# vitskvara/VBMatrixFactorization.jl

Hardware: AMD Instinct MI355X
Metric: VB iterations/sec (higher is better)
Workload: dtype bf16

## Files before the change

### vbmatrixfactorization.jl_amd/csrc/gram_kernels.hpp

```cpp
#pragma once
#include "common.hpp"
#include "ctrl_kernels.hpp"
#include "post_kernels.hpp"

namespace vbmf {

#ifndef GRAM_CHUNK
#define GRAM_CHUNK 256
#endif
constexpr int GRAM_PLANES = 5;
constexpr long long GRAM_G_NT_BYTES = 240LL << 20;

__device__ __forceinline__ unsigned pack_bf2(unsigned short lo, unsigned short hi) { return (unsigned)lo | ((unsigned)hi << 16); }

__global__ __launch_bounds__(256) void gram_build_kernel(const uint4* __restrict__ Y1, int XT, int KS, float* __restrict__ Gt,
                                                         int GT) {
    const int P = blockIdx.y, Q = blockIdx.x;
    if (P > Q) return;
    const int lane = threadIdx.x & 63, w = threadIdx.x >> 6;
    const int p0 = 4 * P + 2 * (w >> 1), q0 = 4 * Q + 2 * (w & 1);
    const long long KT = 2LL * GT;
    double g64[2][2][16];
#pragma unroll
    for (int a = 0; a < 2; ++a)
#pragma unroll
        for (int b = 0; b < 2; ++b)
#pragma unroll
            for (int r = 0; r < 16; ++r) g64[a][b][r] = 0.0;
    const uint4 z = make_uint4(0u, 0u, 0u, 0u);
    const uint4* pa[2];
    const uint4* pb[2];
    bool oka[2], okb[2];
#pragma unroll
    for (int i = 0; i < 2; ++i) {
        oka[i] = p0 + i < XT; okb[i] = q0 + i < XT;
        pa[i] = Y1 + ((long long)(oka[i] ? p0 + i : 0) * KS) * 64 + lane;
        pb[i] = Y1 + ((long long)(okb[i] ? q0 + i : 0) * KS) * 64 + lane;
    }
    constexpr int U = 4;
    for (int k0 = 0; k0 < KS; k0 += GRAM_CHUNK) {
        const int k1 = min(k0 + GRAM_CHUNK, KS);
        f32x16 acc[2][2];
#pragma unroll
        for (int a = 0; a < 2; ++a)
#pragma unroll
            for (int b = 0; b < 2; ++b)
#pragma unroll
                for (int r = 0; r < 16; ++r) acc[a][b][r] = 0.f;
        for (int ks = k0; ks < k1; ks += U) {
            uint4 fa[U][2], fb[U][2];
#pragma unroll
            for (int u = 0; u < U; ++u) {
                const bool in = ks + u < k1;
#pragma unroll
                for (int i = 0; i < 2; ++i) {
                    fa[u][i] = (in && oka[i]) ? pa[i][(long long)(ks + u) * 64] : z;
                    fb[u][i] = (in && okb[i]) ? pb[i][(long long)(ks + u) * 64] : z;
                }
            }
#pragma unroll
            for (int u = 0; u < U; ++u)
#pragma unroll
                for (int a = 0; a < 2; ++a)
#pragma unroll
                    for (int b = 0; b < 2; ++b)
                        acc[a][b] = __builtin_amdgcn_mfma_f32_32x32x16_bf16(__builtin_bit_cast(bf16x8, fa[u][a]),
                                                                            __builtin_bit_cast(bf16x8, fb[u][b]), acc[a][b], 0, 0, 0);
        }
#pragma unroll
        for (int a = 0; a < 2; ++a)
#pragma unroll
            for (int b = 0; b < 2; ++b)
#pragma unroll
                for (int r = 0; r < 16; ++r) g64[a][b][r] += (double)acc[a][b][r];
    }
    const int half = lane >> 5, c = lane & 31;
#pragma unroll
    for (int a = 0; a < 2; ++a)
#pragma unroll
        for (int b = 0; b < 2; ++b) {
            const int p = p0 + a, q = q0 + b;
            if (p > q) continue;
#pragma unroll
            for (int r = 0; r < 16; ++r) {
                const int i = rho(r, half);
                const float v = (float)g64[a][b][r];
                Gt[(((long long)p * KT + 2 * q + (c >> 4)) * 64 + 32 * ((c >> 3) & 1) + i) * 8 + (c & 7)] = v;
                if (p != q) Gt[(((long long)q * KT + 2 * p + (i >> 4)) * 64 + 32 * ((i >> 3) & 1) + c) * 8 + (i & 7)] = v;
            }
        }
}

constexpr int GW_KS = 2, GW_ROWS = 16 * GW_KS;
template <int HP>
__global__ __launch_bounds__(HP * 4) void gram_w_kernel(const float* __restrict__ A32, const float* __restrict__ S,
                                                        const float* __restrict__ Wold, float* __restrict__ Wnew,
                                                        uint4* __restrict__ Wt, long long M, int KT, const int* __restrict__ stop) {
    if (*stop) return;
    constexpr int NS = HP / 16, NH = HP / 32, NT = HP * 4;
    __shared__ float sW[GW_ROWS][HP + 1];
    const int lane = threadIdx.x & 63, cb = threadIdx.x >> 6;
    const int q = lane >> 4, c = lane & 15;
    const long long row0 = (long long)blockIdx.x * GW_ROWS;
    double sb[NS][4];
#pragma unroll
    for (int s = 0; s < NS; ++s)
#pragma unroll
        for (int t = 0; t < 4; ++t) sb[s][t] = (double)S[(long long)(16 * s + 4 * q + t) * HP + 16 * cb + c];
#pragma unroll
    for (int mb = 0; mb < GW_KS; ++mb) {
        const long long m = row0 + 16 * mb + c;
        float4 a[NS];
#pragma unroll
        for (int s = 0; s < NS; ++s)
            a[s] = m < M ? *reinterpret_cast<const float4*>(A32 + m * HP + 16 * s + 4 * q) : make_float4(0.f, 0.f, 0.f, 0.f);
        f64x4 acc = {0.0, 0.0, 0.0, 0.0};
#pragma unroll
        for (int s = 0; s < NS; ++s) {
            acc = __builtin_amdgcn_mfma_f64_16x16x4f64((double)a[s].x, sb[s][0], acc, 0, 0, 0);
            acc = __builtin_amdgcn_mfma_f64_16x16x4f64((double)a[s].y, sb[s][1], acc, 0, 0, 0);
            acc = __builtin_amdgcn_mfma_f64_16x16x4f64((double)a[s].z, sb[s][2], acc, 0, 0, 0);
            acc = __builtin_amdgcn_mfma_f64_16x16x4f64((double)a[s].w, sb[s][3], acc, 0, 0, 0);
        }
#pragma unroll
        for (int r = 0; r < 4; ++r) sW[16 * mb + q + 4 * r][16 * cb + c] = (float)acc[r];
    }
    __syncthreads();
    const long long plane = (long long)KT * NH * 64;
    for (int it = threadIdx.x; it < GW_KS * NH * 64; it += NT) {
        const int jj = it / (NH * 64), ht = (it / 64) % NH, ln = it & 63;
        const int half = ln >> 5, h = 32 * ht + (ln & 31);
        const long long j = (long long)blockIdx.x * GW_KS + jj;
        if (j >= KT) continue;
        unsigned short wp[3][8], dp[2][8];
#pragma unroll
        for (int e = 0; e < 8; ++e) {
            const long long m = 16 * j + 8 * half + e;
            const float wv = sW[16 * jj + 8 * half + e][h];
            const float dv = (float)((double)wv - (double)Wold[m * HP + h]);
            Wnew[m * HP + h] = wv;
            wp[0][e] = f2bf(wv);
            float res = wv - bf2f(wp[0][e]);
            wp[1][e] = f2bf(res);
            res -= bf2f(wp[1][e]);
            wp[2][e] = f2bf(res);
            dp[0][e] = f2bf(dv);
            dp[1][e] = f2bf(dv - bf2f(dp[0][e]));
        }
        const long long o = (j * NH + ht) * 64 + ln;
#pragma unroll
        for (int p = 0; p < 3; ++p)
            Wt[p * plane + o] = make_uint4(pack_bf2(wp[p][0], wp[p][1]), pack_bf2(wp[p][2], wp[p][3]), pack_bf2(wp[p][4], wp[p][5]),
                                           pack_bf2(wp[p][6], wp[p][7]));
#pragma unroll
        for (int p = 0; p < 2; ++p)
            Wt[(3 + p) * plane + o] = make_uint4(pack_bf2(dp[p][0], dp[p][1]), pack_bf2(dp[p][2], dp[p][3]), pack_bf2(dp[p][4], dp[p][5]),
                                                 pack_bf2(dp[p][6], dp[p][7]));
    }
}

template <int HP, int NCG>
__global__ __launch_bounds__(HP * 4 / NCG) void gram_w_cols_kernel(const float* __restrict__ A32, const float* __restrict__ S,
                                                                   const float* __restrict__ Wold, float* __restrict__ Wnew,
                                                                   uint4* __restrict__ Wt, long long M, int KT,
                                                                   const int* __restrict__ stop) {
    if (*stop) return;
    constexpr int NS = HP / 16, NH = HP / 32, HC = HP / NCG, NHC = NH / NCG, NT = HP * 4 / NCG;
    static_assert(HC % 32 == 0 && NT <= 512, "gram_w_cols geometry");
    __shared__ float sW[GW_ROWS][HC + 1];
    const int lane = threadIdx.x & 63, cb = threadIdx.x >> 6;
    const int q = lane >> 4, c = lane & 15;
    const int col0 = blockIdx.y * HC;
    const long long row0 = (long long)blockIdx.x * GW_ROWS;
    double sb[NS][4];
#pragma unroll
    for (int s = 0; s < NS; ++s)
#pragma unroll
        for (int t = 0; t < 4; ++t) sb[s][t] = (double)S[(long long)(16 * s + 4 * q + t) * HP + col0 + 16 * cb + c];
#pragma unroll
    for (int mb = 0; mb < GW_KS; ++mb) {
        const long long m = row0 + 16 * mb + c;
        f64x4 acc = {0.0, 0.0, 0.0, 0.0};
#pragma unroll
        for (int s = 0; s < NS; ++s) {
            const float4 a = m < M ? *reinterpret_cast<const float4*>(A32 + m * HP + 16 * s + 4 * q) : make_float4(0.f, 0.f, 0.f, 0.f);
            acc = __builtin_amdgcn_mfma_f64_16x16x4f64((double)a.x, sb[s][0], acc, 0, 0, 0);
            acc = __builtin_amdgcn_mfma_f64_16x16x4f64((double)a.y, sb[s][1], acc, 0, 0, 0);
            acc = __builtin_amdgcn_mfma_f64_16x16x4f64((double)a.z, sb[s][2], acc, 0, 0, 0);
            acc = __builtin_amdgcn_mfma_f64_16x16x4f64((double)a.w, sb[s][3], acc, 0, 0, 0);
        }
#pragma unroll
        for (int r = 0; r < 4; ++r) sW[16 * mb + q + 4 * r][16 * cb + c] = (float)acc[r];
    }
    __syncthreads();
    const long long plane = (long long)KT * NH * 64;
    for (int it = threadIdx.x; it < GW_KS * NHC * 64; it += NT) {
        const int jj = it / (NHC * 64), htl = (it / 64) % NHC, ln = it & 63;
        const int half = ln >> 5, hl = 32 * htl + (ln & 31), h = col0 + hl, ht = blockIdx.y * NHC + htl;
        const long long j = (long long)blockIdx.x * GW_KS + jj;
        if (j >= KT) continue;
        unsigned short wp[3][8], dp[2][8];
#pragma unroll
        for (int e = 0; e < 8; ++e) {
            const long long m = 16 * j + 8 * half + e;
            const float wv = sW[16 * jj + 8 * half + e][hl];
            const float dv = (float)((double)wv - (double)Wold[m * HP + h]);
            Wnew[m * HP + h] = wv;
            wp[0][e] = f2bf(wv);
            float res = wv - bf2f(wp[0][e]);
            wp[1][e] = f2bf(res);
            res -= bf2f(wp[1][e]);
            wp[2][e] = f2bf(res);
            dp[0][e] = f2bf(dv);
            dp[1][e] = f2bf(dv - bf2f(dp[0][e]));
        }
        const long long o = (j * NH + ht) * 64 + ln;
#pragma unroll
        for (int p = 0; p < 3; ++p)
            Wt[p * plane + o] = make_uint4(pack_bf2(wp[p][0], wp[p][1]), pack_bf2(wp[p][2], wp[p][3]), pack_bf2(wp[p][4], wp[p][5]),
                                           pack_bf2(wp[p][6], wp[p][7]));
#pragma unroll
        for (int p = 0; p < 2; ++p)
            Wt[(3 + p) * plane + o] = make_uint4(pack_bf2(dp[p][0], dp[p][1]), pack_bf2(dp[p][2], dp[p][3]), pack_bf2(dp[p][4], dp[p][5]),
                                                 pack_bf2(dp[p][6], dp[p][7]));
    }
}

__device__ __forceinline__ float sub_f32(float a, float b) {
    float r;
    asm("v_sub_f32 %0, %1, %2" : "=v"(r) : "v"(a), "v"(b));
    return r;
}
__device__ __forceinline__ unsigned cvt_pk_bf16(float lo, float hi) {
    typedef __attribute__((ext_vector_type(2))) float f32x2v;
    typedef __attribute__((ext_vector_type(2))) __bf16 bf16x2v;
    const f32x2v v = {lo, hi};
    return __builtin_bit_cast(unsigned, __builtin_convertvector(v, bf16x2v));
}
__device__ __forceinline__ void split3_frag(const f32x4& x0, const f32x4& x1, u32x4v& g0, u32x4v& g1, u32x4v& g2) {
    const float v[8] = {x0.x, x0.y, x0.z, x0.w, x1.x, x1.y, x1.z, x1.w};
#pragma unroll
    for (int e = 0; e < 4; ++e) {
        float a = v[2 * e], b = v[2 * e + 1];
        const unsigned p0 = cvt_pk_bf16(a, b);
        a = sub_f32(a, bitsf(p0 << 16));
        b = sub_f32(b, bitsf(p0 & 0xffff0000u));
        const unsigned p1 = cvt_pk_bf16(a, b);
        a = sub_f32(a, bitsf(p1 << 16));
        b = sub_f32(b, bitsf(p1 & 0xffff0000u));
        g0[e] = p0;
        g1[e] = p1;
        g2[e] = cvt_pk_bf16(a, b);
    }
}

__device__ __forceinline__ f32x16 mfma_bf(const u32x4v& a, const u32x4v& b, const f32x16& c) {
    return __builtin_amdgcn_mfma_f32_32x32x16_bf16(__builtin_bit_cast(bf16x8, a), __builtin_bit_cast(bf16x8, b), c, 0, 0, 0);
}

#ifndef VBMF_GRAMPROD_PROBE
#define VBMF_GRAMPROD_PROBE 0
#endif
template <int NH>
struct GramProd {
    static constexpr int NW = 8;
    static constexpr int THREADS = 64 * NW;
    static constexpr int TPG = 16 / NH;
    static constexpr int NXW = TPG >= NW ? TPG / NW : 1;
    static constexpr int HS = TPG >= NW ? 1 : NW / TPG;
    static constexpr int NHW = NH / HS;
    static constexpr int CH = NH == 2 ? 4 : 2;
    static constexpr int D = 4;
    static constexpr int U = CH;
    static constexpr int NP = GRAM_PLANES * CH * NH;
    static constexpr int PPW = (NP + NW - 1) / NW;
    static constexpr int GL = 2 * NXW;
    static constexpr int GQ = VBMF_GRAMPROD_PROBE == 2 ? 0 : GL;
    static constexpr int PLANE_BYTES = 2 * NP * 1024;
    static constexpr int RING_BYTES = NW * D * GL * 1024;
    static constexpr int LDS_BYTES = PLANE_BYTES + RING_BYTES;
    static_assert(NXW * (NW / HS) == TPG && NHW * HS == NH, "gram_prod geometry");
    static_assert(LDS_BYTES <= 160 * 1024, "gram_prod LDS");
    static constexpr int g_wait(int u) {
        int n = (D - 1) * GQ;
        for (int d = 1; d < D; ++d) n += ((u + CH * D - d) % CH == 0) ? PPW : 0;
        return n;
    }
};
template <int NH, int NHT = NH>
__global__ __launch_bounds__(GramProd<NH>::THREADS) void gram_prod_kernel(const float4* __restrict__ Gt, const uint4* __restrict__ Wt,
                                                                          float* __restrict__ Out, int GT, int XT1, int sps, int nrg,
                                                                          long long n, long long slab_floats,
                                                                          const int* __restrict__ stop) {
    using C = GramProd<NH>;
    constexpr int NW = C::NW, NXW = C::NXW, NHW = C::NHW, D = C::D, CH = C::CH, U = C::U, NP = C::NP, PPW = C::PPW, GL = C::GL;
    extern __shared__ __attribute__((aligned(1024))) unsigned char gram_lds[];
    if (*stop) return;
    const int lane = threadIdx.x & 63;
    const int w = __builtin_amdgcn_readfirstlane(threadIdx.x >> 6);
    const int rg = blockIdx.x % nrg, s = blockIdx.x / nrg;
    const int KT = 2 * GT;
    const int j0 = s * sps, j1 = min(j0 + sps, KT), nk = j1 - j0;
    const int pt0 = rg * C::TPG + (w % (C::TPG / NXW)) * NXW;
    const int h0 = (w / (C::TPG / NXW)) * NHW;
    const int hg0 = NHT == NH ? 0 : (int)blockIdx.y * NH;
    const long long plane = (long long)KT * NHT * 64;
    f32x16 accP[NXW][NHW], accQ[NXW][NHW];
#pragma unroll
    for (int i = 0; i < NXW; ++i)
#pragma unroll
        for (int h = 0; h < NHW; ++h)
#pragma unroll
            for (int r = 0; r < 16; ++r) { accP[i][h][r] = 0.f; accQ[i][h][r] = 0.f; }
    __amdgpu_buffer_rsrc_t gr[NXW];
#pragma unroll
    for (int i = 0; i < NXW; ++i)
        gr[i] = __builtin_amdgcn_make_buffer_rsrc((void*)(Gt + (long long)(pt0 + i) * KT * 128), 0,
                                                  VBMF_GRAMPROD_PROBE == 1 ? 0u : (unsigned)KT * 2048u, 0x00020000);
    const __amdgpu_buffer_rsrc_t wr = __builtin_amdgcn_make_buffer_rsrc((void*)Wt, 0, (unsigned)(GRAM_PLANES * plane * 16), 0x00020000);
    const int voff = lane * 16;
    unsigned char* const ring = gram_lds + C::PLANE_BYTES + w * (D * GL * 1024);
    const bool g_nt = !(NH == 4 && NHT == 4) && (long long)GT * GT * 4096 > GRAM_G_NT_BYTES;
    auto load_g = [&](int slot, int t) __attribute__((always_inline)) {
        const int so = VBMF_GRAMPROD_PROBE == 3 ? 0 : min(j0 + t, j1 - 1) * 2048;
        if (g_nt) {
#pragma unroll
            for (int i = 0; i < NXW; ++i) {
                lds_dma_piece_nt(gr[i], ring + (slot * GL + 2 * i) * 1024, voff, so);
                lds_dma_piece_nt(gr[i], ring + (slot * GL + 2 * i + 1) * 1024, voff, so + 1024);
            }
        } else {
#pragma unroll
            for (int i = 0; i < NXW; ++i) {
                lds_dma_piece(gr[i], ring + (slot * GL + 2 * i) * 1024, voff, so);
                lds_dma_piece(gr[i], ring + (slot * GL + 2 * i + 1) * 1024, voff, so + 1024);
            }
        }
    };
    auto load_planes = [&](int cc, int t) __attribute__((always_inline)) {
#pragma unroll
        for (int v = 0; v < PPW; ++v) {
            const int x = min(w + NW * v, NP - 1);
            const int q = x / (CH * NH), r = x % (CH * NH);
            const int j = min(j0 + t + r / NH, j1 - 1);
            lds_dma_piece(wr, gram_lds + (cc * NP + x) * 1024, voff, (int)(q * plane + ((long long)j * NHT + hg0 + r % NH) * 64) * 16);
        }
    };
#pragma unroll
    for (int d = 0; d < D; ++d) {
        if ((d + CH * D - D) % CH == 0) load_planes(0, 0);
        load_g(d, d);
    }
    asm volatile("s_waitcnt vmcnt(%0)" ::"n"(CH * GL) : "memory");
    __builtin_amdgcn_s_barrier();
    asm volatile("" ::: "memory");
    u32x4v wf[GRAM_PLANES][NHW], g[NXW][3];
    auto mma = [&]() __attribute__((always_inline)) {
#pragma unroll
        for (int i = 0; i < NXW; ++i) {
#pragma unroll
            for (int h = 0; h < NHW; ++h) {
                f32x16 a = accP[i][h];
                a = mfma_bf(wf[2][h], g[i][0], a);
                a = mfma_bf(wf[1][h], g[i][1], a);
                a = mfma_bf(wf[0][h], g[i][2], a);
                a = mfma_bf(wf[1][h], g[i][0], a);
                a = mfma_bf(wf[0][h], g[i][1], a);
                accP[i][h] = mfma_bf(wf[0][h], g[i][0], a);
                f32x16 d = accQ[i][h];
                d = mfma_bf(wf[4][h], g[i][0], d);
                d = mfma_bf(wf[3][h], g[i][1], d);
                accQ[i][h] = mfma_bf(wf[3][h], g[i][0], d);
            }
        }
    };
    int slot = 0;
    auto body = [&](int t0, bool tail) __attribute__((always_inline)) {
#pragma unroll
        for (int u = 0; u < U; ++u) {
            const int t = t0 + u, kk = u % CH;
            const int cc = (t / CH) & 1;
            const bool live = !tail || t < nk;
            asm volatile("s_waitcnt vmcnt(%0)" ::"n"(C::g_wait(u)) : "memory");
            if (live) {
                const unsigned char* gs = ring + slot * (GL * 1024) + lane * 32;
                f32x4 x[NXW][2];
#pragma unroll
                for (int i = 0; i < NXW; ++i) {
                    x[i][0] = *reinterpret_cast<const f32x4*>(gs + i * 2048);
                    x[i][1] = *reinterpret_cast<const f32x4*>(gs + i * 2048 + 16);
                }
                const unsigned char* pl = gram_lds + (cc * NP + kk * NH + h0) * 1024 + lane * 16;
#pragma unroll
                for (int q = 0; q < GRAM_PLANES; ++q)
#pragma unroll
                    for (int h = 0; h < NHW; ++h) wf[q][h] = *reinterpret_cast<const u32x4v*>(pl + (q * CH * NH + h) * 1024);
#pragma unroll
                for (int i = 0; i < NXW; ++i) split3_frag(x[i][0], x[i][1], g[i][0], g[i][1], g[i][2]);
            }
            __builtin_amdgcn_sched_barrier(0);
            if (kk == 0) load_planes(cc ^ 1, t + CH);
            if (VBMF_GRAMPROD_PROBE != 2) load_g(slot, t + D);
            slot = slot + 1 == D ? 0 : slot + 1;
            __builtin_amdgcn_sched_barrier(0);
            if (live) mma();
            if (kk == CH - 1) {
                asm volatile("s_waitcnt vmcnt(%0) lgkmcnt(0)" ::"n"(CH * C::GQ) : "memory");
                __builtin_amdgcn_s_barrier();
                asm volatile("" ::: "memory");
            }
        }
    };
    int t0 = 0;
    for (; t0 + U <= nk; t0 += U) body(t0, false);
    if (t0 < nk) body(t0, true);
    asm volatile("s_waitcnt vmcnt(0)" ::: "memory");
    float4* oP = reinterpret_cast<float4*>(Out + (long long)s * slab_floats);
    float4* oQ = reinterpret_cast<float4*>(Out + (long long)s * slab_floats + n);
#pragma unroll
    for (int i = 0; i < NXW; ++i) {
        const int p = pt0 + i;
        if (p >= XT1) continue;
#pragma unroll
        for (int h = 0; h < NHW; ++h) {
            const long long o = (((long long)p * NHT + hg0 + h0 + h) * 64 + lane) * 4;
            const f32x16 a = accP[i][h], d = accQ[i][h];
#pragma unroll
            for (int q = 0; q < 4; ++q) {
                oP[o + q] = float4{a[4 * q], a[4 * q + 1], a[4 * q + 2], a[4 * q + 3]};
                oQ[o + q] = float4{d[4 * q], d[4 * q + 1], d[4 * q + 2], d[4 * q + 3]};
            }
        }
    }
}

template <int HP>
struct GPart {
    static constexpr int V = HP / 16, S = 8 / V, NH = HP / 32;
    static constexpr int NT = 512, SD = 8;
    static constexpr int PPT = HP == 128 ? 2 : 3;
    static constexpr int ROWS = PPT * NT * 4 / HP;
    static constexpr int NSTEP = ROWS / 4 / S;
    static constexpr int BUF = ROWS * HP;
    static constexpr int SU = V == 8 ? 2 : 4;
    static_assert(NSTEP % SU == 0 && (ROWS / 4) % S == 0 && ROWS % 16 == 0, "gram_tail geometry");
    static_assert((S - 1) * V * V * 64 * 32 <= 2 * BUF * 4, "gram_tail: the subset fold reuses the block buffers");
};
template <int HP>
__device__ __forceinline__ int gpart_index(int a, int b) {
    constexpr int V = GPart<HP>::V;
    const int tw = a % V, i = a / V, t = b % V, c = b / V;
    return ((((tw * V + t) * 4 + (i >> 2)) << 6) + 16 * (i & 3) + c);
}
__device__ __forceinline__ void add4(float4& s, const float4& v) { s.x += v.x; s.y += v.y; s.z += v.z; s.w += v.w; }
struct GTailRound { float4 a0, a1, a2, a3, a4, a5, a6, a7; };
__device__ __forceinline__ void gtail_load(GTailRound& v, const __amdgpu_buffer_rsrc_t (&r)[8], int voff, int cnt) {
    const auto ld = [&](int u) __attribute__((always_inline)) {
        return __builtin_bit_cast(float4, __builtin_amdgcn_raw_buffer_load_b128(r[u], voff, 0, 0));
    };
    switch (cnt) {
        default: v.a7 = ld(7); [[fallthrough]];
        case 7: v.a6 = ld(6); [[fallthrough]];
        case 6: v.a5 = ld(5); [[fallthrough]];
        case 5: v.a4 = ld(4); [[fallthrough]];
        case 4: v.a3 = ld(3); [[fallthrough]];
        case 3: v.a2 = ld(2); [[fallthrough]];
        case 2: v.a1 = ld(1); [[fallthrough]];
        case 1: v.a0 = ld(0);
    }
}
template <bool FIRST>
__device__ __forceinline__ float4 gtail_sum(const GTailRound& v, float4 f, int cnt) {
    if (FIRST) f = v.a0;
    else add4(f, v.a0);
    if (cnt > 1) add4(f, v.a1);
    if (cnt > 2) add4(f, v.a2);
    if (cnt > 3) add4(f, v.a3);
    if (cnt > 4) add4(f, v.a4);
    if (cnt > 5) add4(f, v.a5);
    if (cnt > 6) add4(f, v.a6);
    if (cnt > 7) add4(f, v.a7);
    return f;
}
template <int HP, int HPT>
struct GPartBlk {
    static constexpr int NQ = HPT / HP;
    static constexpr long long STRIDE = 2LL * HPT * HPT + (NQ == 1 ? 1 : NQ);
};
template <int HP, int HPT = HP>
__global__ __launch_bounds__(512) void gram_tail_kernel(const float* slabs, int nslab, long long slab_floats, float* PQ, long long n,
                                                        long long Mp1, const float* __restrict__ Wn, const float* __restrict__ Wo,
                                                        const float* __restrict__ A32, long long M, int rpc, int nchunk,
                                                        double* __restrict__ part, const int* __restrict__ stop) {
    using C = GPart<HP>;
    constexpr int V = C::V, S = C::S, NH = C::NH, PPT = C::PPT, SD = C::SD, ROWS = C::ROWS, NSTEP = C::NSTEP, SU = C::SU;
    constexpr int NQ = GPartBlk<HP, HPT>::NQ, NHT = HPT / 32;
    constexpr bool BLK = NQ > 1;
    constexpr long long STRIDE = GPartBlk<HP, HPT>::STRIDE;
    static_assert(HPT % HP == 0, "gram_tail blocks");
    __shared__ __attribute__((aligned(32))) float stage[2 * C::BUF];
    __shared__ double red[8];
    const int stopv = *stop;
    const int lane = threadIdx.x & 63;
    const int w = __builtin_amdgcn_readfirstlane(threadIdx.x >> 6);
    const int s = w / V, tw = w % V;
    const int q = lane >> 4, c = lane & 15;
    const unsigned cp = BLK ? blockIdx.x / (NQ * NQ) : blockIdx.x;
    const int qa = BLK ? (blockIdx.x / NQ) % NQ : 0, qb = BLK ? blockIdx.x % NQ : 0;
    const int chunk = cp >> 1, pi = cp & 1;
    const long long m0 = (long long)chunk * rpc, m1 = min(m0 + rpc, M);
    const long long fend = chunk == nchunk - 1 ? Mp1 : m0 + rpc;
    const float* src = slabs + (pi ? n : 0);
    float* dst = PQ + (pi ? n : 0);
    const float* X = pi ? Wo : A32;
    const int xr = lane >> 2, r4 = lane & 3;
    int grp[PPT], ht[PPT], half[PPT];
#pragma unroll
    for (int j = 0; j < PPT; ++j) {
        const int sg = 8 * j + w;
        grp[j] = sg / (2 * NH);
        ht[j] = (sg % (2 * NH)) >> 1;
        half[j] = sg & 1;
    }
    GTailRound v[PPT];
    static_assert(SD == 8, "gram_tail: GTailRound");
    float wv[NSTEP], xv[NSTEP];
    auto piece_off = [&](long long rb, int j) __attribute__((always_inline)) {
        const long long row = rb + 16 * grp[j] + xr;
        return ((((row >> 5) * NHT + qb * NH + ht[j]) * 64 + half[j] * 32 + (row & 31)) << 4) + 4 * r4;
    };
    auto issue_slabs = [&](long long rb, int k0) __attribute__((always_inline)) {
        __amdgpu_buffer_rsrc_t r[SD];
#pragma unroll
        for (int u = 0; u < SD; ++u)
            r[u] = __builtin_amdgcn_make_buffer_rsrc((void*)(src + (long long)(k0 + u) * slab_floats), 0, (unsigned)(n * 4), 0x00020000);
#pragma unroll
        for (int j = 0; j < PPT; ++j) {
            if (rb + 16 * grp[j] >= fend) continue;
            gtail_load(v[j], r, (int)(piece_off(rb, j) * 4), min(SD, nslab - k0));
        }
    };
    auto fold_slabs = [&](long long rb, int k0, float4 (&f)[PPT]) __attribute__((always_inline)) {
#pragma unroll
        for (int j = 0; j < PPT; ++j) {
            if (rb + 16 * grp[j] >= fend) continue;
            if (k0 == 0) f[j] = gtail_sum<true>(v[j], f[j], min(SD, nslab));
            else f[j] = gtail_sum<false>(v[j], f[j], min(SD, nslab - k0));
        }
    };
    const __amdgpu_buffer_rsrc_t wr = __builtin_amdgcn_make_buffer_rsrc((void*)Wn, 0, (unsigned)(m1 * HPT * 4), 0x00020000);
    const __amdgpu_buffer_rsrc_t xd = __builtin_amdgcn_make_buffer_rsrc((void*)X, 0, (unsigned)(m1 * HPT * 4), 0x00020000);
    auto issue_w = [&](long long rb) __attribute__((always_inline)) {
        const int o = (int)(((rb + 4 * s + q) * HPT + qa * HP + V * c + tw) * 4);
#pragma unroll
        for (int i = 0; i < NSTEP; ++i) {
            wv[i] = bitsf(__builtin_amdgcn_raw_buffer_load_b32(wr, o + i * (4 * S * HPT * 4), 0, 0));
            xv[i] = bitsf(__builtin_amdgcn_raw_buffer_load_b32(xd, o + i * (4 * S * HPT * 4), 0, 0));
        }
    };
    issue_slabs(m0, 0);
    issue_w(m0);
    if (stopv) return;
    f64x4 acc[V];
#pragma unroll
    for (int t = 0; t < V; ++t) acc[t] = f64x4{0.0, 0.0, 0.0, 0.0};
    double tr = 0.0;
    int buf = 0;
    for (long long rb = m0; rb < fend; rb += ROWS, buf ^= 1) {
        float* sb = stage + buf * C::BUF;
        float4 f[PPT];
        fold_slabs(rb, 0, f);
        for (int k0 = SD; k0 < nslab; k0 += SD) {
            issue_slabs(rb, k0);
            fold_slabs(rb, k0, f);
        }
#pragma unroll
        for (int j = 0; j < PPT; ++j) {
            if (rb + 16 * grp[j] >= fend) continue;
            if (nslab > 1 && (!BLK || qa == 0)) *reinterpret_cast<float4*>(dst + piece_off(rb, j)) = f[j];
            *reinterpret_cast<float4*>(sb + (16 * grp[j] + xr) * HP + 32 * ht[j] + 8 * r4 + 4 * half[j]) = f[j];
        }
        float ac[NSTEP], xc[NSTEP];
#pragma unroll
        for (int i = 0; i < NSTEP; ++i) {
            xc[i] = xv[i];
            ac[i] = pi ? (float)((double)wv[i] - (double)xc[i]) : wv[i];
        }
        if (rb + ROWS < fend) {
            issue_slabs(rb + ROWS, 0);
            issue_w(rb + ROWS);
        }
        asm volatile("s_waitcnt lgkmcnt(0)" ::: "memory");
        __builtin_amdgcn_s_barrier();
        asm volatile("" ::: "memory");
#pragma unroll
        for (int i0 = 0; i0 < NSTEP; i0 += SU) {
            if (rb + 4 * (s + S * i0) >= m1) break;
            __builtin_amdgcn_sched_barrier(0);
#pragma unroll
            for (int i = i0; i < i0 + SU; ++i) {
                const int rl = 4 * (s + S * i) + q;
                const bool in = rb + rl < m1;
                float pv[V];
                if constexpr (V == 2) {
                    const float2 x = *reinterpret_cast<const float2*>(sb + rl * HP + 2 * c);
                    pv[0] = x.x; pv[1] = x.y;
                } else {
#pragma unroll
                    for (int g = 0; g < V / 4; ++g) {
                        const float4 x = *reinterpret_cast<const float4*>(sb + rl * HP + V * c + 4 * g);
                        pv[4 * g] = x.x; pv[4 * g + 1] = x.y; pv[4 * g + 2] = x.z; pv[4 * g + 3] = x.w;
                    }
                }
#pragma unroll
                for (int t = 0; t < V; ++t) pv[t] = in ? pv[t] : 0.f;
                if (!pi && (!BLK || qa == qb)) {
                    float p = 0.f;
#pragma unroll
                    for (int t = 0; t < V; ++t) p = t == tw ? pv[t] : p;
                    tr += (double)xc[i] * (double)p;
                }
#pragma unroll
                for (int t = 0; t < V; ++t) acc[t] = __builtin_amdgcn_mfma_f64_16x16x4f64((double)ac[i], (double)pv[t], acc[t], 0, 0, 0);
            }
        }
    }
    if constexpr (S > 1) {
        f64x4* fold = reinterpret_cast<f64x4*>(stage);
        __syncthreads();
        if (s > 0) {
#pragma unroll
            for (int t = 0; t < V; ++t) fold[(((s - 1) * V + tw) * V + t) * 64 + lane] = acc[t];
        }
        __syncthreads();
        if (s == 0) {
            for (int s2 = 1; s2 < S; ++s2)
#pragma unroll
                for (int t = 0; t < V; ++t) acc[t] += fold[(((s2 - 1) * V + tw) * V + t) * 64 + lane];
        }
    }
    double* o = part + (long long)chunk * STRIDE + pi * HPT * HPT + (qa * NQ + qb) * HP * HP;
    if (s == 0) {
#pragma unroll
        for (int t = 0; t < V; ++t)
#pragma unroll
            for (int r = 0; r < 4; ++r) o[(((tw * V + t) * 4 + r) << 6) + lane] = acc[t][r];
    }
    if (pi || (BLK && qa != qb)) return;
    for (int off = 32; off > 0; off >>= 1) tr += __shfl_down(tr, off);
    if (lane == 0) red[w] = tr;
    __syncthreads();
    if (threadIdx.x == 0) {
        double t = 0.0;
        for (int i = 0; i < 8; ++i) t += red[i];
        part[(long long)chunk * STRIDE + 2 * HPT * HPT + qa] = t;
    }
}

constexpr int GRED_E = 64, GRED_G = 4;
template <int DP>
__device__ __forceinline__ void gred_round(const double* __restrict__ part, int k, int nchunk, long long stride, long long i0,
                                           long long i1, double& s0, double& s1) {
    double v0[DP], v1[DP];
#pragma unroll
    for (int u = 0; u < DP; ++u) {
        const long long o = (long long)min(k + u * GRED_G, nchunk - 1) * stride;
        v0[u] = part[o + i0];
        v1[u] = part[o + i1];
    }
    __builtin_amdgcn_sched_barrier(0);
#pragma unroll
    for (int u = 0; u < DP; ++u)
        if (k + u * GRED_G < nchunk) { s0 += v0[u]; s1 += v1[u]; }
}
template <int HP, int HPT = HP>
__global__ __launch_bounds__(256) void gram_part_reduce_kernel(const double* __restrict__ part, int nchunk, double* __restrict__ st,
                                                               StateLayout lay, const int* __restrict__ stop) {
    const int stopv = *stop;
    constexpr int V = GPart<HP>::V, n2 = HPT * HPT, nb = HP * HP, NQ = GPartBlk<HP, HPT>::NQ;
    constexpr bool BLK = NQ > 1;
    static_assert(NQ <= 2, "gram_part_reduce: two trace slots");
    constexpr long long stride = GPartBlk<HP, HPT>::STRIDE;
    __shared__ double sum[2][GRED_G][GRED_E];
    const int el = threadIdx.x % GRED_E, g = threadIdx.x / GRED_E;
    const int e = blockIdx.x * GRED_E + el;
    const int pi = e / n2, blk = BLK ? (e % n2) / nb : 0, x = BLK ? e % nb : e % n2;
    const int qa = blk / NQ, qb = blk % NQ;
    const int tw = (x >> 8) / V, t = (x >> 8) % V, rq = (x >> 6) & 3, q = (x >> 4) & 3, c = x & 15;
    const int al = V * (q + 4 * rq) + tw, bl = V * c + t;
    const int a = qa * HP + al, b = qb * HP + bl;
    const bool mat = e < 2 * n2, tro = e == 2 * n2;
    const long long i0 = mat ? e : 2LL * n2;
    const long long i1 = mat ? (long long)pi * n2 + (qb * NQ + qa) * nb + gpart_index<HP>(bl, al) : 2LL * n2 + (BLK ? 1 : 0);
    double s0 = 0.0, s1 = 0.0;
    for (int k = g; k < nchunk; k += 32 * GRED_G) {
        const int left = (nchunk - k + GRED_G - 1) / GRED_G;
        if (left <= 8) gred_round<8>(part, k, nchunk, stride, i0, i1, s0, s1);
        else if (left <= 16) gred_round<16>(part, k, nchunk, stride, i0, i1, s0, s1);
        else gred_round<32>(part, k, nchunk, stride, i0, i1, s0, s1);
    }
    if (stopv) return;
    sum[0][g][el] = s0;
    sum[1][g][el] = s1;
    __syncthreads();
    if (g != 0 || !(mat || tro)) return;
    double t0 = 0.0, t1 = 0.0;
    for (int k = 0; k < GRED_G; ++k) { t0 += sum[0][k][el]; t1 += sum[1][k][el]; }
    if (tro) st[lay.GX()] = BLK ? t0 + t1 : t0;
    else st[(pi ? lay.GD() : lay.GB()) + a * HPT + b] = 0.5 * (t0 + t1);
}

}
```

Baseline: 4898.

## Add phased ping-pong wave scheduling to gram product kernel for NH=2

For the NH=2 instantiation, the two halves of the workgroup's waves are offset by one barrier phase. Each k-step is split into a load phase and an MFMA phase separated by block barriers, so one half issues memory/LDS work while the other half runs matrix instructions. The goal is to stagger memory and MFMA pressure across waves for better overlap, at the cost of two extra barriers per k-step. It also adds optional s_memtime timestamp instrumentation, which is compiled out by default.

```diff
diff --git a/vbmatrixfactorization.jl_amd/csrc/gram_kernels.hpp b/vbmatrixfactorization.jl_amd/csrc/gram_kernels.hpp
--- a/vbmatrixfactorization.jl_amd/csrc/gram_kernels.hpp
+++ b/vbmatrixfactorization.jl_amd/csrc/gram_kernels.hpp
@@ -261,8 +261,26 @@
 #ifndef VBMF_GRAMPROD_PROBE
 #define VBMF_GRAMPROD_PROBE 0
 #endif
+#ifndef VBMF_GRAMPROD_STAMPS
+#define VBMF_GRAMPROD_STAMPS 0
+#endif
+#ifndef VBMF_GRAMPROD_STAMP_T0
+#define VBMF_GRAMPROD_STAMP_T0 8
+#endif
+constexpr int GRAM_STAMP_T0 = VBMF_GRAMPROD_STAMP_T0, GRAM_STAMP_WGS = 3, GRAM_STAMP_KS = 4;
+#if VBMF_GRAMPROD_STAMPS
+__device__ unsigned long long gram_prod_stamp_buf[GRAM_STAMP_WGS * 8 * GRAM_STAMP_KS * 4];
+extern "C" int vbmf_gram_prod_stamps(unsigned long long* dst) {
+    return (int)hipMemcpyFromSymbol(dst, HIP_SYMBOL(gram_prod_stamp_buf), sizeof(gram_prod_stamp_buf));
+}
+#endif
 template <int NH>
 struct GramProd {
+#ifdef VBMF_GRAMPROD_PHASED
+    static constexpr bool PH = VBMF_GRAMPROD_PHASED != 0;
+#else
+    static constexpr bool PH = NH == 2;
+#endif
     static constexpr int NW = 8;
     static constexpr int THREADS = 64 * NW;
     static constexpr int TPG = 16 / NH;
@@ -375,12 +393,25 @@
         }
     };
     int slot = 0;
+#if VBMF_GRAMPROD_STAMPS
+    static_assert(U <= GRAM_STAMP_KS, "gram_prod stamps");
+    unsigned long long stamp[GRAM_STAMP_KS][4] = {};
+#define GRAM_STAMP(u, k) do { if (t0 == GRAM_STAMP_T0) stamp[u][k] = __builtin_amdgcn_s_memtime(); } while (0)
+#else
+#define GRAM_STAMP(u, k) do { } while (0)
+#endif
+    const bool second = w >= NW / 2;
+    if (C::PH) {
+        if (second) __builtin_amdgcn_s_barrier();
+        asm volatile("" ::: "memory");
+    }
     auto body = [&](int t0, bool tail) __attribute__((always_inline)) {
 #pragma unroll
         for (int u = 0; u < U; ++u) {
             const int t = t0 + u, kk = u % CH;
             const int cc = (t / CH) & 1;
             const bool live = !tail || t < nk;
+            GRAM_STAMP(u, 0);
             asm volatile("s_waitcnt vmcnt(%0)" ::"n"(C::g_wait(u)) : "memory");
             if (live) {
                 const unsigned char* gs = ring + slot * (GL * 1024) + lane * 32;
@@ -403,7 +434,27 @@
             if (VBMF_GRAMPROD_PROBE != 2) load_g(slot, t + D);
             slot = slot + 1 == D ? 0 : slot + 1;
             __builtin_amdgcn_sched_barrier(0);
+            if (C::PH) {
+                if (kk == CH - 1) asm volatile("s_waitcnt vmcnt(%0) lgkmcnt(0)" ::"n"(CH * C::GQ) : "memory");
+                else asm volatile("s_waitcnt lgkmcnt(0)" ::: "memory");
+                GRAM_STAMP(u, 1);
+                __builtin_amdgcn_s_barrier();
+                asm volatile("" ::: "memory");
+                __builtin_amdgcn_sched_barrier(0);
+                GRAM_STAMP(u, 2);
+                if (live) mma();
+                __builtin_amdgcn_sched_barrier(0);
+                GRAM_STAMP(u, 3);
+                asm volatile("s_waitcnt lgkmcnt(0)" ::: "memory");
+                __builtin_amdgcn_s_barrier();
+                asm volatile("" ::: "memory");
+                __builtin_amdgcn_sched_barrier(0);
+                continue;
+            }
+            GRAM_STAMP(u, 1);
+            GRAM_STAMP(u, 2);
             if (live) mma();
+            GRAM_STAMP(u, 3);
             if (kk == CH - 1) {
                 asm volatile("s_waitcnt vmcnt(%0) lgkmcnt(0)" ::"n"(CH * C::GQ) : "memory");
                 __builtin_amdgcn_s_barrier();
@@ -432,6 +483,13 @@
             }
         }
     }
+    if (C::PH && !second) __builtin_amdgcn_s_barrier();
+#if VBMF_GRAMPROD_STAMPS
+    const int sw = blockIdx.x == 0 ? 0 : blockIdx.x == 1 ? 1 : blockIdx.x == gridDim.x / 2 ? 2 : -1;
+    if (sw >= 0 && blockIdx.y == 0 && lane < GRAM_STAMP_KS * 4)
+        gram_prod_stamp_buf[(sw * NW + w) * (GRAM_STAMP_KS * 4) + lane] = stamp[lane / 4][lane % 4];
+#endif
+#undef GRAM_STAMP
 }
 
 template <int HP>
```

After: 4882, median of 2. Within noise of the previous version (-0.3%).
